# srihari-humbarwadi/retinanet-tensorflow2.x

Hardware: AMD Instinct MI355X
Metric: images/sec train, ResNet50-640 RetinaNet data-parallel step (encode + fwd + loss + bwd + clip + all-reduce + SGD/EMA); inference images/s under `infer` (higher is better)
Workload: dtype bf16; 1 GPU; ResNet50-640x640 bf16 training, 32 images/GPU (BASELINE configs[2] shard: global batch 32), resnet_initial frozen, single GPU; global_batch=32, parallelism=dp1, rccl_ranks=1, comm=torch, syncbn_messages=0

## Files before the change

### include/rnet_hip.h

```cpp
#ifndef RNET_HIP_H_
#define RNET_HIP_H_

#include <stddef.h>
#include <stdint.h>

#ifdef __cplusplus
extern "C" {
#endif
#if defined(__GNUC__)
#pragma GCC visibility push(default)
#endif

typedef enum {
  RN_OK = 0,
  RN_EINVAL = -1,
  RN_ENOMEM = -2,
  RN_EHIP = -3,
  RN_ECOMM = -4,
  RN_EUNSUPPORTED = -5
} rn_status;

enum { RN_DT_F32 = 0, RN_DT_BF16 = 1 };
enum { RN_ACT_NONE = 0, RN_ACT_RELU = 1, RN_ACT_RELU6 = 2, RN_ACT_SWISH = 3 };
enum { RN_FUSION_FAST_ATTENTION = 1, RN_FUSION_FAST_CHANNEL_ATTENTION = 2 };
// ... 100 lines not shown

typedef struct {
  const void* x;
  const void* w;
  void* y;
  const float* scale;
  const float* shift;
  const void* residual;
  int32_t N, H, W, Cin, pix_stride, Ho, Wo, Cout;
  float* bn_partial;
  const float* bias;
  int32_t w_terms;
  int32_t w_pair;
  const void* bn_bwd_y;
  const float* bn_bwd_fwd;
} rn_conv_segment;

typedef struct {
  int32_t R, S, stride_h, stride_w, pad_top, pad_left;
  int32_t act;
  int32_t out_dtype;
  int32_t num_segments;
  rn_conv_segment seg[RN_CONV_MAX_SEGMENTS];
  rn_launch_opts opts;
  void* splitk_ws;
  int64_t splitk_ws_bytes;
} rn_conv_problem;

int rn_conv2d_nhwc_fwd(const rn_conv_problem* problem , void* stream);
size_t rn_conv_splitk_workspace_bytes(const rn_conv_problem* problem );
// ... 271 lines not shown
```

### retinanet-tensorflow2.x_amd/csrc/rn_conv.hip

```cpp
#include "rn_conv_dev.h"

template <int BM, int BN, int BK, bool OUT_F32, int STAGES, bool SPLIT>
__global__ void __launch_bounds__(CONV_THREADS, 2) conv_fwd_kernel(const ConvArgs args) {
  static_assert((STAGES >= 3 && STAGES <= 8) || STAGES == 32, "no K loop for this stage count");
  constexpr int WM = 2, WN = 2;
  constexpr int NWAVES = WM * WN;
  constexpr int NTHREADS = 64 * NWAVES;
  constexpr int SLOTS = BK / 8;
  constexpr int RPI = 64 / SLOTS;
  constexpr int A_INSTR = BM / RPI / NWAVES;
  constexpr int B_INSTR = BN / RPI / NWAVES;
  constexpr int WTM = BM / WM, WTN = BN / WN;
  constexpr int TM = WTM / 32, TN = WTN / 32;
  constexpr int KSUB = BK / 16;
  constexpr int A_BYTES = BM * BK * 2, B_BYTES = BN * BK * 2;
  constexpr int STAGE_BYTES = A_BYTES + B_BYTES;
  static_assert(A_INSTR >= 1 && B_INSTR >= 1, "tile too small for the wave count");

  extern __shared__ __attribute__((aligned(16))) char smem[];

  int tile, part = 0;
  {
    const int total = SPLIT ? args.vtotal : args.total_tiles;
    const int bid = blockIdx.x;
// ... 346 lines not shown
        }
#pragma unroll
        for (int q = 0; q < 4; ++q) {
          float t = f4[q] + sbs[q];
          if (round1) t = rn_rb(t);
          if (affine) t = t * ssc[q] + ssf[q];
          if (round2) t = rn_rb(t);
          f4[q] = t;
        }
        v = make_float4(f4[0], f4[1], f4[2], f4[3]);
      } else {
        v = *(const float4*)(cl + rr * BN + ec);
      }
      const long long o = (long long)m * Cout + n;
      if (sg.residual) {
        const uint2 rv = *(const uint2*)(sg.residual + o);
        v.x += rn_bf16_to_f32((uint16_t)(rv.x & 0xffffu));
        v.y += rn_bf16_to_f32((uint16_t)(rv.x >> 16));
        v.z += rn_bf16_to_f32((uint16_t)(rv.y & 0xffffu));
        v.w += rn_bf16_to_f32((uint16_t)(rv.y >> 16));
      }
      {
        float f4[4] = {v.x, v.y, v.z, v.w};
        if (!OUT_F32 && args.act == RN_ACT_SWISH) {
#pragma unroll
          for (int q = 0; q < 4; ++q) f4[q] = rn_rb(f4[q]);
        }
        rn_apply_act_n<4>(f4, args.act);
        v = make_float4(f4[0], f4[1], f4[2], f4[3]);
      }
      if (OUT_F32) {
// ... 253 lines not shown
```

### retinanet-tensorflow2.x_amd/csrc/rn_conv_big_epi.h

```cpp
#ifndef RN_CONV_BIG_EPI_H_
#define RN_CONV_BIG_EPI_H_
#include <type_traits>

#include "rn_conv_dev.h"

#ifdef HALO_PROF
__device__ unsigned long long g_halo_clk[48];
#define EPI_STAMP(k_) if (blockIdx.x == 0 && threadIdx.x == 0) g_halo_clk[k_] = clock64();
#else
#define EPI_STAMP(k_)
#endif

#ifdef HALO_ABLATE
#define EPI_ABLATE HALO_ABLATE
#else
#define EPI_ABLATE 0
#endif

typedef rn_h16 bf16x2_t __attribute__((ext_vector_type(2)));
typedef float f32x2_t __attribute__((ext_vector_type(2)));

__device__ __forceinline__ uint32_t pack2(float lo, float hi) {
  f32x2_t v = {lo, hi};
  bf16x2_t b = __builtin_convertvector(v, bf16x2_t);
  return __builtin_bit_cast(uint32_t, b);
}
typedef short i16x2_t __attribute__((ext_vector_type(2)));
__device__ __forceinline__ uint32_t pk_max_i16(uint32_t a, uint32_t b) {
  return __builtin_bit_cast(uint32_t, __builtin_elementwise_max(__builtin_bit_cast(i16x2_t, a), __builtin_bit_cast(i16x2_t, b)));
}
__device__ __forceinline__ uint32_t pk_min_i16(uint32_t a, uint32_t b) {
  return __builtin_bit_cast(uint32_t, __builtin_elementwise_min(__builtin_bit_cast(i16x2_t, a), __builtin_bit_cast(i16x2_t, b)));
}
__device__ __forceinline__ float bf_lo(uint32_t u) { return rn_lo16(u); }
__device__ __forceinline__ float bf_hi(uint32_t u) { return rn_hi16(u); }

__device__ __forceinline__ int tile_of(int v, int total) {
  const int xcd = v & 7, slot = v >> 3;
  const int q = total >> 3, r = total & 7;
  return (xcd < r ? xcd * (q + 1) : r * (q + 1) + (xcd - r) * q) + slot;
}

template <bool OUT_F32, bool HAS_RES>
__device__ __forceinline__ bool big_bias_in_acc(const ConvArgs& args, const ConvSegDev& sg) {
  if (HAS_RES) return false;
  return sg.bias != nullptr;
}
template <bool OUT_F32, bool HAS_RES, int WM = 2>
__device__ __forceinline__ void big_acc_init(f32x16_t (&acc)[4][2], const ConvArgs& args, int c_si, int c_n0, int wave,
                                             bool with_bias = true) {
// ... 131 lines not shown
    }
#pragma unroll
    for (int q = 0; q < 8; ++q) asm volatile("" : "+v"(sc[q]), "+v"(sf[q]));
    if (BN_BWD) {
#pragma unroll
      for (int q = 0; q < 8; ++q) asm volatile("" : "+v"(mu[q]), "+v"(is[q]));
    }
    EPI_STAMP(12);
    const bool has_res = HAS_RES && sg.residual != nullptr;
    const uint16_t* const side = BN_BWD ? sg.bn_y : sg.residual;
    const bool has_side = BN_BWD ? true : has_res;
    const bool stats = sg.bn_partial != nullptr;
    float st0[8], st1[8];
#pragma unroll
    for (int q = 0; q < 8; ++q) st0[q] = st1[q] = 0.0f;
    char* const ybase = (char*)sg.y + ((long long)(mw0 + rrow) * Cout + nr) * 2;
    const long long row_bytes = (long long)Cout * 2;
    const int act = args.act;
    const bool clamp_lo = act == RN_ACT_RELU || act == RN_ACT_RELU6, clamp_hi = act == RN_ACT_RELU6;
    const bool affine = !BN_BWD && (sg.scale != nullptr || sg.shift != nullptr);
    const bool plain = BN_BWD || (!affine && !has_res && act != RN_ACT_SWISH);
    const bool round2 = affine && has_res;
    uint4 rv[2][LOADS ? 4 : 1];
#define BIG_RES_PREFETCH(buf_, i_)                                                                    \
_Pragma("unroll") for (int pass = 0; pass < (LOADS ? 4 : 0); ++pass) {                              \
  const int m = mw0 + (i_) * 32 + pass * 8 + rrow;                                                  \
  rv[buf_][pass] = make_uint4(0u, 0u, 0u, 0u);                                                      \
  if (has_side && nok && m < M) rv[buf_][pass] = *(const uint4*)(side + (long long)m * Cout + nr);  \
}
    const uint32_t lo2 = clamp_lo ? 0u : 0x80008000u, hi2 = clamp_hi ? RN_SIX_X2 : 0x7fff7fffu;
    auto blocks = [&](auto plain_c, auto stats_c, auto round2_c, auto swish_c) __attribute__((always_inline)) {
      constexpr bool PLAIN = decltype(plain_c)::value;
      constexpr int STATS = decltype(stats_c)::value, ROUND2 = decltype(round2_c)::value, SWISH = decltype(swish_c)::value;
      BIG_RES_PREFETCH(0, 0);
#pragma unroll
      for (int i = 0; i < 4; ++i) {
        EPI_STAMP(13 + 2 * i);
        if (i + 1 < 4) BIG_RES_PREFETCH((i + 1) & 1, i + 1);
        if (FROM_WS) big_epi_rebuild<2>(&acc[i][0], src, i, 0);
#pragma unroll
        for (int j = 0; j < 2; ++j)
#pragma unroll
          for (int g = 0; g < 4; ++g) {
            const int nl = j * 32 + g * 8 + fh * 4;
            uint2 pk;
            pk.x = pack2(acc[i][j][g * 4 + 0], acc[i][j][g * 4 + 1]);
            pk.y = pack2(acc[i][j][g * 4 + 2], acc[i][j][g * 4 + 3]);
            *(uint2*)(patch + fr * 128 + (((nl >> 3) ^ (fr & 7)) << 4) + ((((nl >> 2) ^ (fr >> 3)) & 1) << 3)) = pk;
          }
        EPI_STAMP(14 + 2 * i);
        uint4 vb[4];
#pragma unroll
        for (int pass = 0; pass < 4; ++pass) {
          const int row = pass * 8 + rrow;
          const uint4 t = *(const uint4*)(patch + row * 128 + ((ru ^ (row & 7)) << 4));
          vb[pass] = (pass & 1) ? make_uint4(t.z, t.w, t.x, t.y) : t;
        }
#pragma unroll
        for (int pass = 0; pass < 4; ++pass) {
          const int row = pass * 8 + rrow;
          const uint4 v = vb[pass];
          const int m = mw0 + i * 32 + row;
          if (m < M && nok) {
            uint4 ov;
            if (PLAIN) {
              ov.x = pk_min_i16(pk_max_i16(v.x, lo2), hi2); ov.y = pk_min_i16(pk_max_i16(v.y, lo2), hi2);
              ov.z = pk_min_i16(pk_max_i16(v.z, lo2), hi2); ov.w = pk_min_i16(pk_max_i16(v.w, lo2), hi2);
            } else {
              const uint4 r4 = HAS_RES ? rv[i & 1][LOADS ? pass : 0] : make_uint4(0u, 0u, 0u, 0u);
              float f[8] = {bf_lo(v.x), bf_hi(v.x), bf_lo(v.y), bf_hi(v.y), bf_lo(v.z), bf_hi(v.z), bf_lo(v.w), bf_hi(v.w)};
              const float rr[8] = {bf_lo(r4.x), bf_hi(r4.x), bf_lo(r4.y), bf_hi(r4.y),
                                   bf_lo(r4.z), bf_hi(r4.z), bf_lo(r4.w), bf_hi(r4.w)};
#pragma unroll
              for (int q = 0; q < 8; ++q) f[q] = f[q] * sc[q] + sf[q];
              if (ROUND2 == 1 || (ROUND2 == 2 && round2)) {
#pragma unroll
                for (int q = 0; q < 8; q += 2) {
                  const uint32_t pq = pack2(f[q], f[q + 1]);
                  f[q] = bf_lo(pq); f[q + 1] = bf_hi(pq);
                }
              }
#pragma unroll
              for (int q = 0; q < 8; ++q) f[q] += rr[q];
              if (SWISH == 1 || (SWISH == 2 && act == RN_ACT_SWISH)) {
#pragma unroll
                for (int q = 0; q < 8; ++q) f[q] = rn_swish(rn_rb(f[q]));
              }
              ov.x = pack2(f[0], f[1]); ov.y = pack2(f[2], f[3]); ov.z = pack2(f[4], f[5]); ov.w = pack2(f[6], f[7]);
              ov.x = pk_min_i16(pk_max_i16(ov.x, lo2), hi2); ov.y = pk_min_i16(pk_max_i16(ov.y, lo2), hi2);
              ov.z = pk_min_i16(pk_max_i16(ov.z, lo2), hi2); ov.w = pk_min_i16(pk_max_i16(ov.w, lo2), hi2);
            }
            if (!(EPI_ABLATE & 16) || ov.x == 0x12345678u) *(uint4*)(ybase + (long long)(i * 32 + pass * 8) * row_bytes) = ov;
            if (STATS == 1 || (STATS == 2 && stats)) {
              const float w[8] = {bf_lo(ov.x), bf_hi(ov.x), bf_lo(ov.y), bf_hi(ov.y),
                                  bf_lo(ov.z), bf_hi(ov.z), bf_lo(ov.w), bf_hi(ov.w)};
              if (BN_BWD) {
                const uint4 y4 = rv[i & 1][LOADS ? pass : 0];
                const float yy[8] = {bf_lo(y4.x), bf_hi(y4.x), bf_lo(y4.y), bf_hi(y4.y),
                                     bf_lo(y4.z), bf_hi(y4.z), bf_lo(y4.w), bf_hi(y4.w)};
#pragma unroll
                for (int q = 0; q < 8; ++q) {
                  const float g = (yy[q] * sc[q] + sf[q]) > 0.0f ? w[q] : 0.0f;
                  st0[q] += g;
                  st1[q] += g * ((yy[q] - mu[BN_BWD ? q : 0]) * is[BN_BWD ? q : 0]);
                }
              } else {
#pragma unroll
                for (int q = 0; q < 8; ++q) { st0[q] += w[q]; st1[q] += w[q] * w[q]; }
              }
            }
          }
        }
      }
    };
    typedef std::integral_constant<int, 0> off_t;
    typedef std::integral_constant<int, 1> on_t;
    typedef std::integral_constant<int, 2> runtime_t;
    if constexpr (BN_BWD) {
      blocks(std::true_type{}, on_t{}, off_t{}, off_t{});
    } else if (plain) {
      if (stats) blocks(std::true_type{}, on_t{}, off_t{}, off_t{});
      else blocks(std::true_type{}, off_t{}, off_t{}, off_t{});
    } else if (!stats && act != RN_ACT_SWISH) {
      if (round2) blocks(std::false_type{}, off_t{}, on_t{}, off_t{});
      else blocks(std::false_type{}, off_t{}, off_t{}, off_t{});
    } else {
      blocks(std::false_type{}, runtime_t{}, runtime_t{}, runtime_t{});
    }
    EPI_STAMP(21);
    if (stats) {
#pragma unroll
      for (int q = 0; q < 8; ++q) {
#pragma unroll
        for (int o = 8; o < 64; o <<= 1) {
          st0[q] += __shfl_xor(st0[q], o, 64);
          st1[q] += __shfl_xor(st1[q], o, 64);
        }
      }
      if (rrow == 0 && nok) {
        float* dst = sg.bn_partial + ((long long)(chunk0 >= 0 ? chunk0 : c_m0 / 128) + wave_m) * 2 * Cout + nr;
        *(float4*)(dst) = make_float4(st0[0], st0[1], st0[2], st0[3]);
        *(float4*)(dst + 4) = make_float4(st0[4], st0[5], st0[6], st0[7]);
// ... 58 lines not shown
```

### retinanet-tensorflow2.x_amd/csrc/rn_conv_dev.h

```cpp
#ifndef RN_CONV_DEV_H_
#define RN_CONV_DEV_H_
#include "rn_common.h"

typedef rn_h16 bf16x8_t __attribute__((ext_vector_type(8)));
typedef float f32x16_t __attribute__((ext_vector_type(16)));

#define CONV_THREADS 256

struct ConvSegDev {
  const uint16_t* x;
  const uint16_t* w;
  void* y;
  const float* scale;
  const float* shift;
  const uint16_t* residual;
  float* bn_partial;
  const float* bias;
  const uint16_t* bn_y;
  const float* bn_fwd;
  int N, H, W, Cin, pix_stride, Ho, Wo, Cout;
  int M, tile_begin, n_tiles, CinP;
  int cwrap, halo_pitch;
  int pair_cout, rows;
};


struct ConvArgs {
  int R, S, sh, sw, pt, pl, act, nseg, total_tiles, pad_;
  int split_f, split_s, vtotal, pad2_;
  float* ws;
  ConvSegDev seg[RN_CONV_MAX_SEGMENTS];
};

#define RN_SPLITK_HEADER_BYTES 16384
// ... 30 lines not shown
```

### retinanet-tensorflow2.x_amd/csrc/rn_conv_dispatch.hip

```cpp
#include <algorithm>
#include <map>
#include <mutex>
#include <tuple>

#include "rn_conv_dev.h"

extern "C" int rn_conv_cout_pad(int Cout) { return Cout <= 64 ? 64 : (int)rn_align_up((size_t)Cout, 128); }
extern "C" int rn_conv_cin_pad(int Cin) { return Cin <= 32 ? 32 : (int)rn_align_up((size_t)Cin, 64); }
extern "C" int rn_conv_pair_rows(int Cout) { return Cout > 0 ? 128 * ((Cout + 63) / 64) : 0; }

struct ConvPlanSeg {
  int cols, cols_pad;
  int terms, cin_pad;
  long long M;
  int n_tiles, tile_begin;
  int bn_row_blocks;
};

struct ConvPlan {
  int kid;
  int BM, BN;
  int BK;
  int bal_rows;
  bool deal;
// ... 212 lines not shown
    RN_CHECK_ARG(s.Cout % 4 == 0, "rn_conv2d_nhwc_fwd: segment %d Cout=%d not a multiple of 4", i, s.Cout);
    RN_CHECK_ARG((pl.seg[i].cols_pad <= 64) == (pl.seg[0].cols_pad <= 64), "rn_conv2d_nhwc_fwd: segments mix Cout tile widths");
    RN_CHECK_ARG(!s.w_pair || (pl.kid != 0 && p->out_dtype == RN_DT_F32 && s.w_terms <= 1 && !s.scale && !s.shift &&
                               !s.residual && !s.bn_partial),
                 "rn_conv2d_nhwc_fwd: segment %d: w_pair needs an f32 launch without scale / shift / residual that the 256- / "
                 "512-row kernels take (rn_conv_kernel_id() != 0)", i);
    RN_CHECK_ARG(((uintptr_t)s.x | (uintptr_t)s.w | (uintptr_t)s.y | (uintptr_t)s.residual) % 16 == 0,
                 "rn_conv2d_nhwc_fwd: segment %d tensors must be 16-byte aligned", i);
    RN_CHECK_ARG(pl.seg[i].M < (1ll << 31) && (long long)s.N * s.H * s.W * s.pix_stride * 2 < (1ll << 31),
                 "rn_conv2d_nhwc_fwd: segment %d input exceeds the 2 GiB buffer-addressing limit", i);
    if (s.bn_bwd_y) {
      RN_CHECK_ARG(s.bn_partial && s.bn_bwd_fwd && p->out_dtype == RN_DT_BF16 && !s.scale && !s.shift && !s.bias &&
                       !s.residual && p->act == RN_ACT_NONE && s.Cout % 8 == 0 && (uintptr_t)s.bn_bwd_y % 16 == 0,
                   "rn_conv2d_nhwc_fwd: segment %d: bn_bwd_y needs bn_partial + bn_bwd_fwd on a plain bf16 launch", i);
    }
    RN_CHECK_ARG((s.bn_bwd_y != nullptr) == (p->seg[0].bn_bwd_y != nullptr),
                 "rn_conv2d_nhwc_fwd: bn_bwd_y must be set on all segments or none");
    RN_CHECK_ARG(pl.seg[i].terms <= 3, "rn_conv2d_nhwc_fwd: segment %d w_terms=%d (1..3)", i, s.w_terms);
  }
  RN_CHECK_ARG(p->splitk_ws == nullptr || ((uintptr_t)p->splitk_ws % 16 == 0 && p->splitk_ws_bytes >= 0),
               "rn_conv2d_nhwc_fwd: splitk_ws must be 16-byte aligned");
  return RN_OK;
}

extern "C" int rn_conv2d_nhwc_fwd(const rn_conv_problem* p, void* stream) {
  RN_CHECK_ARG(p != nullptr, "rn_conv2d_nhwc_fwd: null problem");
  RN_CHECK_ARG(p->num_segments >= 1 && p->num_segments <= RN_CONV_MAX_SEGMENTS,
               "rn_conv2d_nhwc_fwd: num_segments=%d", p->num_segments);
  ConvPlan pl;
  conv_plan(p, false, pl);
// ... 2 lines not shown
  ConvArgs a;
  a.R = p->R; a.S = p->S; a.sh = p->stride_h; a.sw = p->stride_w; a.pt = p->pad_top; a.pl = p->pad_left;
  a.act = p->act; a.nseg = p->num_segments;
  a.total_tiles = (int)pl.total_tiles;
  a.pad_ = pl.kid <= 1 ? (pl.fast_div ? 1 : 0) | (pl.deal ? 2 : 0) : 0;
  a.split_f = a.vtotal = a.total_tiles; a.split_s = 1; a.pad2_ = 0; a.ws = nullptr;
  for (int ii = 0; ii < p->num_segments; ++ii) {
    const rn_conv_segment& s = p->seg[pl.order[ii]];
    const ConvPlanSeg& ps = pl.seg[pl.order[ii]];
    ConvSegDev& d = a.seg[ii];
    d.x = (const uint16_t*)s.x; d.w = (const uint16_t*)s.w; d.y = s.y;
    d.scale = s.scale; d.shift = s.shift; d.residual = (const uint16_t*)s.residual;
    d.bn_partial = s.bn_partial;
    d.bn_y = (const uint16_t*)s.bn_bwd_y;
    d.bn_fwd = s.bn_bwd_fwd;
    d.bias = s.bias;
    d.N = s.N; d.H = s.H; d.W = s.W; d.Cin = s.Cin; d.pix_stride = s.pix_stride;
    d.Ho = s.Ho; d.Wo = s.Wo; d.Cout = ps.cols;
    d.pair_cout = s.w_pair ? s.Cout : 0;
    d.rows = pl.bal_rows;
    d.M = (int)ps.M;
    d.tile_begin = ps.tile_begin;
    d.n_tiles = ps.n_tiles;
    d.cwrap = ps.cin_pad;
    d.CinP = ps.terms * ps.cin_pad;
    d.halo_pitch = s.W + 1;
  }

  hipStream_t st = (hipStream_t)stream;
  const bool f32 = p->out_dtype == RN_DT_F32;
// ... 13 lines not shown
```

### retinanet-tensorflow2.x_amd/csrc/rn_core.hip

```cpp
#include "rn_common.h"
#include <string.h>
#include <new>

static thread_local char g_rn_err[512] = "";

void rn_set_error(const char* fmt, ...) {
  va_list ap;
  va_start(ap, fmt);
  vsnprintf(g_rn_err, sizeof(g_rn_err), fmt, ap);
  va_end(ap);
}

extern "C" const char* rn_last_error(void) { return g_rn_err; }

extern "C" int rn_abi_version(void) { return 13; }

extern "C" int rn_storage_dtype(void) {
#ifdef RN_F16
  return 1;
#else
  return 0;
#endif
}

extern "C" int rn_device_ok(void) {
  int n = 0;
  if (hipGetDeviceCount(&n) != hipSuccess || n <= 0) {
    (void)hipGetLastError();
    return 0;
  }
// ... 122 lines not shown
```

### retinanet-tensorflow2.x_amd/retinanet/_C.py

```python
from __future__ import annotations

import ctypes
import logging
import os
from ctypes import (POINTER, Structure, c_char_p, c_float, c_int, c_int32, c_int64, c_longlong, c_size_t, c_uint32,
                    c_uint64, c_void_p)

_HERE = os.path.dirname(os.path.abspath(__file__))
LIB_PATH = os.environ.get("RNET_HIP_LIB") or os.path.join(_HERE, "librnet_hip.so")
LIB_PATH_F16 = os.environ.get("RNET_HIP_LIB_F16") or os.path.join(_HERE, "librnet_hip_f16.so")

RN_DT_F32, RN_DT_BF16 = 0, 1
RN_OK, RN_EINVAL, RN_ENOMEM, RN_EHIP, RN_ECOMM, RN_EUNSUPPORTED = 0, -1, -2, -3, -4, -5
RN_ACT_NONE, RN_ACT_RELU, RN_ACT_RELU6, RN_ACT_SWISH = 0, 1, 2, 3
RN_FUSION_FAST_ATTENTION, RN_FUSION_FAST_CHANNEL_ATTENTION = 1, 2
FUSION_IDS = {"fast_attention": RN_FUSION_FAST_ATTENTION, "fast_channel_attention": RN_FUSION_FAST_CHANNEL_ATTENTION}
RN_CONV_MAX_SEGMENTS = 10
ABI_VERSION = 13
RN_OPT_ADAM, RN_OPT_RMSPROP, RN_OPT_ADAGRAD, RN_OPT_SGD = 1, 2, 3, 4
RN_OPT_AMSGRAD, RN_OPT_CENTERED, RN_OPT_MOMENTUM, RN_OPT_NESTEROV = 1, 2, 4, 8
PRED_W_TERMS = int(os.environ.get("RNET_PRED_W_TERMS", "2"))
ACT_IDS = {None: RN_ACT_NONE, "none": RN_ACT_NONE, "relu": RN_ACT_RELU, "relu6": RN_ACT_RELU6,
           "swish": RN_ACT_SWISH}


class RnetError(RuntimeError):
    pass


class DgradPack(Structure):
    _fields_ = [("w_ohwi", c_void_p), ("w_packed", c_void_p), ("R", c_int32), ("S", c_int32), ("Cin", c_int32),
                ("Cout", c_int32), ("Cout_pad", c_int32), ("pad_", c_int32)]

# ... 26 lines not shown
class OptimRule(Structure):
    _fields_ = [("rule", c_int32), ("flags", c_int32), ("lr", c_float), ("beta1", c_float), ("beta2", c_float),
                ("rho", c_float), ("momentum", c_float), ("epsilon", c_float), ("ema_decay", c_float)]


class Bottleneck64Problem(Structure):
    _fields_ = [("x", c_void_p), ("y", c_void_p), ("w_packed", c_void_p), ("affine", c_void_p), ("N", c_int32), ("H", c_int32),
                ("W", c_int32), ("Cx", c_int32), ("opts", LaunchOpts)]


class ConvSegment(Structure):
    _fields_ = [("x", c_void_p), ("w", c_void_p), ("y", c_void_p), ("scale", c_void_p), ("shift", c_void_p),
                ("residual", c_void_p), ("N", c_int32), ("H", c_int32), ("W", c_int32), ("Cin", c_int32),
                ("pix_stride", c_int32), ("Ho", c_int32), ("Wo", c_int32), ("Cout", c_int32), ("bn_partial", c_void_p),
                ("bias", c_void_p), ("w_terms", c_int32), ("w_pair", c_int32), ("bn_bwd_y", c_void_p),
                ("bn_bwd_fwd", c_void_p)]


class ConvProblem(Structure):
    _fields_ = [("R", c_int32), ("S", c_int32), ("stride_h", c_int32), ("stride_w", c_int32),
                ("pad_top", c_int32), ("pad_left", c_int32), ("act", c_int32), ("out_dtype", c_int32),
                ("num_segments", c_int32), ("seg", ConvSegment * RN_CONV_MAX_SEGMENTS), ("opts", LaunchOpts),
                ("splitk_ws", c_void_p), ("splitk_ws_bytes", c_int64)]


class WgradSegment(Structure):
    _fields_ = [("x", c_void_p), ("dy", c_void_p), ("N", c_int32), ("H", c_int32), ("W", c_int32),
                ("Cin", c_int32), ("Ho", c_int32), ("Wo", c_int32), ("Cout", c_int32),
                ("dy_pix_stride", c_int32), ("x_pix_stride", c_int32)]


# ... 411 lines not shown
```

### retinanet-tensorflow2.x_amd/retinanet/model/train_engine.py

```python
from __future__ import annotations

import ctypes
import os
from typing import NamedTuple

import numpy as np
import torch

from retinanet import _C
from .bottleneck import Bottleneck64, fused_blocks
from .data_parallel import GradientOverlap, SmallMessages
from .forward import (FoldedConvs, FusionState, conv_launch_name, conv_problem, dw_problem, fold_bn, half_activations, maxpool_step,
                      output_view, padded_outputs, split_by_depth, stem_input, stem_pool_partner, stem_pool_step, stem_problem, tensor_readers,
                      topdown_step)

_DT = {"bf16": torch.bfloat16, "f32": torch.float32}
_SEG_DTYPE = np.dtype([("offset", "<i8"), ("size", "<i8"), ("wd", "<i4"), ("bb", "<i4"), ("nb", "<i4"),
                       ("pad", "<i4"), ("bf", "<i8")])


def _hwio_to_ohwi(w):
    return w.permute(3, 0, 1, 2).contiguous()


# ... 12 lines not shown
    frozen: bool = False


class BackwardStep:
    __slots__ = ("run", "side", "writes", "wgrad")

    def __init__(self, run, side=False, writes=(), wgrad=None):
        self.run, self.side, self.writes, self.wgrad = run, side, writes, wgrad

    def __call__(self, st):
        return self.run(st)


class TrainEngine:
    def __init__(self, model, batch_size, frozen_regexes=(), process_group=None, world_size=None, frozen_names=(),
                 launch_opts=None, wide_pred_terms=None, force_dp=None):
        self.model = model
        self.g = model.graph
        self.params_cfg = model.params
        self.B = int(batch_size)
        self.dev = model.device
        env = os.environ.get
        if force_dp is None:
            force_dp = env("RNET_FORCE_DP", "0") == "1"
        if wide_pred_terms is None:
            wide_pred_terms = env("RNET_TRAIN_PRED_W_TERMS") or \
                getattr(getattr(model.params, "training", None), "prediction_weight_planes", None) or 2
        comm_cus = int(env("RNET_COMM_CUS", "8"))
        self.fuse_bn_stats = env("RNET_FUSE_BN_STATS", "1") != "0"
        self.fuse_bn_bwd = env("RNET_FUSE_BN_BWD", "1") != "0"
        self.fuse_bn_bwd_groups = env("RNET_FUSE_BN_BWD", "1") == "2"
        self.side_stream_on = env("RNET_WGRAD_STREAM", "1") != "0"
        cus = env("RNET_WGRAD_CUS", "160,208")
        self._wgrad_cap = tuple(int(v) for v in cus.split(",")) if cus not in ("0", "") else None
        if not self.side_stream_on:
            self._wgrad_cap = None
        if self._wgrad_cap and len(self._wgrad_cap) == 1:
            self._wgrad_cap = (self._wgrad_cap[0], 2 * self._wgrad_cap[0])
        self._wgrad_group_mode = env("RNET_WGRAD_GROUP", "halo")
        self._ab_workspaces = env("RNET_AB_WORKSPACES") == "1"
        self.f16 = half_activations(model.params)
        self.h16 = torch.float16 if self.f16 else torch.bfloat16
        self._DT = {"bf16": self.h16, "f32": torch.float32}
        self.lib = _C.lib(self.f16)
# ... 499 lines not shown
    def _conv_meta(self, p):
        osz = 4 if p.out_dtype == _C.RN_DT_F32 else 2
        dom = True
        for i in range(p.num_segments):
            s = p.seg[i]
            dom = dom and s.Cout > 64 and s.Cin % 64 == 0 and p.out_dtype == _C.RN_DT_BF16
        if id(p) in self._algo:
            flops, byts = self._algo[id(p)]
        else:
            flops = byts = 0
            for i in range(p.num_segments):
                s = p.seg[i]
                flops += 2 * s.N * s.Ho * s.Wo * p.R * p.S * s.Cin * s.Cout
                byts += 2 * s.N * s.H * s.W * s.pix_stride + osz * s.N * s.Ho * s.Wo * s.Cout + 2 * p.R * p.S * s.Cin * s.Cout
                if s.residual:
                    byts += 2 * s.N * s.Ho * s.Wo * s.Cout
        variant = None
        kid = self.lib.rn_conv_kernel_id(ctypes.byref(p))
        has_res = any(p.seg[i].residual for i in range(p.num_segments))
        bnb = bool(p.seg[0].bn_bwd_y)
        tmpl = (f"<{'true' if p.out_dtype == _C.RN_DT_F32 else 'false'}, {'true' if has_res else 'false'}, "
                f"{'true' if bnb else 'false'}>")
        if kid == 2:
            variant = "conv_halo_kernel" + tmpl[:-1] + ", false, 2> (256x256x32, 3x3 halo patch)"
        elif kid == 3:
            variant = "conv_halo_kernel" + tmpl[:-1] + ", false, 4> (512x128x32, 3x3 halo patch)"
        elif kid == 1:
            variant = "conv_big_kernel" + tmpl + " (256x256x32)"
        elif dom:
            variant = "conv_fwd_kernel<128,128,64,bf16>"
        return flops, byts, variant
# ... 322 lines not shown
        lib, B = self.lib, self.B
        self.bwd_steps = []
        self.dgrad_packs = []
        ops = self.ops
        self.dw_flip_packs = []
        plan, done = [], set()
        for op in ops:
            if op["op"] in ("conv", "dwconv"):
                launch = self._launch_ops(op, done)
                if launch:
                    plan.append((op["op"], launch))
            elif op["op"] in ("maxpool", "topdown", "balance", "stem", "se"):
                plan.append((op["op"], op))
        plan.reverse()
        written = set()

        def mark(name):
            first = name not in written
            written.add(name)
            return first

        for kind, item in plan:
            if kind == "conv":
                self._plan_conv_backward(item, mark)
            elif kind == "dwconv":
                self._plan_dw_backward(item, mark)
            elif kind == "se":
                op = item
                x, dy, dx = self.t[op["inp"]], self.grad[op["out"]], self.grad[op["inp"]]
                mark(op["inp"])
                name, se = op["se"], self.g.ses[op["se"]]
                a = (x.data_ptr(), dy.data_ptr(), dx.data_ptr(), B, x.shape[1] * x.shape[2], se["C"],
                     self.Pbf.data_ptr() + 2 * self.bf_off[name + ":w1"],
                     self.Pbf.data_ptr() + 2 * self.bf_off[name + ":w2"], se["se"], self.se_state[op["out"]].data_ptr(),
                     self._pview(name + "/conv2d/kernel", self.G).data_ptr(),
# ... 67 lines not shown
                op = item
                names = op["tensors"]
                dout = [self.grad["bal:" + n] for n in names]
                ins = [self.t[n] for n in names]
                din = [self.grad[n] for n in names]
                for n in names:
                    mark(n)
                nsc = lib.rn_balance_features_bwd_scratch_bytes(len(names), op["mid"], B, ins[0].shape[1], ins[0].shape[2],
                                                                ins[0].shape[3])
                scratch = torch.empty((max(int(nsc), 256),), dtype=torch.uint8, device=self.dev)
                pd, pi, pn = _C.ptr_array(dout), _C.ptr_array(ins), _C.ptr_array(din)
                self._keep += [pd, pi, pn, scratch]
                a = (pd, pi, pn, self.bal_avg.data_ptr(), scratch.data_ptr(), scratch.numel(), len(names), op["mid"], B,
                     ins[0].shape[1], ins[0].shape[2], ins[0].shape[3])
                self.bwd_steps.append(BackwardStep(lambda st, a=a: _C.check(lib.rn_balance_features_bwd(*a, st), "balance_bwd")))
        self._launch_names = {id(q): n for n, q in self.conv_launches}
        self._loss_dy = {k: {lv: self.dy_of[name] for lv, name in self.g.outputs[k].items() if name in self.dy_of}
                         for k in self.g.outputs}
        if self.dgrad_packs:
            arr = (_C.DgradPack * len(self.dgrad_packs))()
            for i, (mptr, k, cin, cout, cw, buf, mode) in enumerate(self.dgrad_packs):
                arr[i].w_ohwi, arr[i].w_packed = mptr, buf.data_ptr()
                arr[i].R, arr[i].S, arr[i].Cin, arr[i].Cout, arr[i].Cout_pad, arr[i].pad_ = k, k, cin, cout, cw, mode
            self._dgrad_pack_items = arr

    def _plan_fused_topdown_backward(self, op, act, mark):
        lib, B, fus = self.lib, self.B, self.fusion_state[id(op)]
        L = len(op["ins"])
        prev_g = prev_coef = None
        for l in range(L):
# ... 146 lines not shown
    def _plan_conv_backward(self, ops, mark):
        lib, B = self.lib, self.B
        if not self._conv_trainable(ops[0]) and not any(self.requires.get(o["inp"]) for o in ops):
            return
        if not self._conv_trainable(ops[0]):
            raise NotImplementedError("backward through a frozen conv that sits above trainable layers")
        live_bn = bool(self._bn_trainable(ops[0]))
        frozen_bn = self._bn_frozen(ops[0])
        if live_bn or frozen_bn:
            grp = self.bn_groups[ops[0]["out"]]
            pb = grp.problem
            for i, op in enumerate(ops):
                s = pb.seg[i]
                s.dz = self.grad[op["out"]].data_ptr()
                if op.get("residual") and self.requires.get(op["residual"]):
                    dres, first = self._grad_target(op["residual"], mark, balanced=False)
                    s.dres, s.dres_accumulate = dres.data_ptr(), 0 if first else 1
            if frozen_bn:
                self.bwd_steps.append(self._bn_frozen_bwd_step(grp))
            else:
                self.bwd_steps.append(self._bn_bwd_step(grp, self.bn_bwd_ws.get(id(pb), grp.ws)))
            dy_of = {op["out"]: grp.dys[i] for i, op in enumerate(ops)}
        else:
            dy_of = {}
            for op in ops:
                if op["out_dtype"] == "f32":
                    shp = list(self.t[op["out"]].shape)
                    shp[3] = (shp[3] + 63) // 64 * 64
                    dyb = torch.zeros(shp, dtype=self.h16, device=self.dev)
                    dy_of[op["out"]] = dyb
# ... 141 lines not shown
                gbuf, first = self._grad_target(op["inp"], mark)
                s = p.seg[i]
                s.x, s.w, s.y = src.data_ptr(), flips[op["dw"]].data_ptr(), gbuf.data_ptr()
                s.scale, s.shift = None, None
                s.residual = None if first else gbuf.data_ptr()
                s.N, s.H, s.W, s.C, s.Ho, s.Wo = B, H, W, d["C"], H, W
            self._keep.append(p)
            self.dw_launches.append(("dw_dgrad:" + "+".join(o["out"] for o in sub), "dgrad", p, ups))

            def dgrad(st, p=p, ups=ups):
                for u in ups:
                    _C.check(lib.rn_upsample_zero2x(*u, st), "rn_upsample_zero2x")
                _C.check(lib.rn_depthwise_conv2d_nhwc_fwd(ctypes.byref(p), st), "dw dgrad")
            self.bwd_steps.append(BackwardStep(dgrad))

    def _bn_bwd_fusable(self, name):
        if not self.fuse_bn_bwd or name in self.bal_src or len(self.readers.get(name, [])) != 1:
            return None
        hit = self._bn_of_tensor.get(name)
        if hit is None:
            return None
        pb, i, o, nseg = hit
        if nseg != 1 and not self.fuse_bn_bwd_groups:
            return None
        if (o["op"] != "conv" or o.get("act") != "relu" or o.get("residual") or
                o.get("survival") is not None or not self._bn_trainable(o) or pb.seg[i].sample_scale):
            return None
        return pb, i

    def _fuse_bn_bwd(self, p, need):
# ... 55 lines not shown
            c = self.g.convs[op["conv"]]
            cin = c["cin"]
            dy = dy_of[op["out"]]
            cw = dy.shape[3]
            cwp = lib.rn_conv_cin_pad(cw)
            if op["conv"] not in packs:
                shape = (lib.rn_conv_cout_pad(4 * cin), 2, 2, cwp) if subpixel else (lib.rn_conv_cout_pad(cin), k, k, cwp)
                packs[op["conv"]] = torch.empty(shape, dtype=self.h16, device=self.dev)
                off, _ = self.p_off[c.get("kvar", op["conv"] + "/kernel")]
                self.dgrad_packs.append((self.P.data_ptr() + 4 * off, k, cin, c["cout"], cwp, packs[op["conv"]],
                                         1 if subpixel else 0))
            x = self._src(op["inp"])
            H, W = x.shape[1], x.shape[2]
            gbuf, first = self._grad_target(op["inp"], mark)
            firsts.append(first)
            src, dst, cout, res = dy, gbuf, cin, None
            if subpixel:
                cout = 4 * cin
                dst = torch.empty((B, dy.shape[1], dy.shape[2], cout), dtype=self.h16, device=self.dev)
                post.append((dst.data_ptr(), gbuf.data_ptr(), B, dy.shape[1], dy.shape[2], cin, 0 if first else 1))
            elif lowres:
                dst = torch.empty((B, dy.shape[1], dy.shape[2], cin), dtype=self.h16, device=self.dev)
                post.append((dst.data_ptr(), gbuf.data_ptr(), B, dy.shape[1], dy.shape[2], cin, H, W, 0 if first else 1))
            else:
                if stride == 2:
                    src, up_args = self._zero_upsampled(dy, H, W)
                    ups.append(up_args)
                res = None if first else gbuf.data_ptr()
            if dst is not gbuf:
                self._keep.append(dst)
            s = p.seg[i]
            s.x, s.w, s.y = src.data_ptr(), packs[op["conv"]].data_ptr(), dst.data_ptr()
            s.scale, s.shift, s.residual = None, None, res
            s.N, s.H, s.W, s.Cin, s.pix_stride = B, src.shape[1], src.shape[2], cw, cw
            s.Ho, s.Wo, s.Cout = dst.shape[1], dst.shape[2], cout
            Ho, Wo = self.tensors[op["out"]][:2]
            fl += 2 * B * Ho * Wo * k * k * cin * c["cout"]
            by += 2 * B * Ho * Wo * c["cout"] + 2 * B * H * W * cin * (2 if res else 1) + 2 * k * k * cin * c["cout"]
        if post_op is None and stride == 1 and all(firsts):
            by += self._fuse_bn_bwd(p, need)
        self._algo[id(p)] = (fl, by)
        self._keep.append(p)
        self.conv_launches.append(("dgrad:" + (need[0].get("group") or need[0]["out"]), p))

        def dgrad(st, p=p, ups=ups, post=post):
            for u in ups:
                _C.check(lib.rn_upsample_zero2x(*u, st), "rn_upsample_zero2x")
            self._launch_conv(p, st, "dgrad")
            for a in post:
                _C.check(post_op[0](*a, st), post_op[1])
        self.bwd_steps.append(BackwardStep(dgrad))

    def refresh_dgrad_weights(self, st):
# ... 255 lines not shown
```

Before: 1139 images/s.

## Fold gated skip-connection gradient into the stride-1 dgrad conv epilogue

For identity skip connections with a ReLU join, the residual-branch gradient is no longer written separately by the BN backward. Instead the downstream dgrad conv epilogue reads the join gradient, masks it with the ReLU activation bitmask, and adds it as a residual. This removes a separate gradient write and accumulate pass over the skip tensor. The cost is extra gate-bit loads and DPP shuffles in the epilogue, new template variants, and stricter planning constraints enforced with asserts.

```diff
diff --git a/include/rnet_hip.h b/include/rnet_hip.h
--- a/include/rnet_hip.h
+++ b/include/rnet_hip.h
@@ -138,6 +138,7 @@
   int32_t w_pair;
   const void* bn_bwd_y;
   const float* bn_bwd_fwd;
+  const uint8_t* residual_gate;
 } rn_conv_segment;
 
 typedef struct {
diff --git a/retinanet-tensorflow2.x_amd/csrc/rn_conv.hip b/retinanet-tensorflow2.x_amd/csrc/rn_conv.hip
--- a/retinanet-tensorflow2.x_amd/csrc/rn_conv.hip
+++ b/retinanet-tensorflow2.x_amd/csrc/rn_conv.hip
@@ -384,7 +384,12 @@
       }
       const long long o = (long long)m * Cout + n;
       if (sg.residual) {
-        const uint2 rv = *(const uint2*)(sg.residual + o);
+        uint2 rv = *(const uint2*)(sg.residual + o);
+        if (!OUT_F32 && sg.res_gate) {
+          const uint32_t bits = (uint32_t)sg.res_gate[o >> 3] >> (n & 4);
+          rv.x &= ((bits & 1u) ? 0xffffu : 0u) | ((bits & 2u) ? 0xffff0000u : 0u);
+          rv.y &= ((bits & 4u) ? 0xffffu : 0u) | ((bits & 8u) ? 0xffff0000u : 0u);
+        }
         v.x += rn_bf16_to_f32((uint16_t)(rv.x & 0xffffu));
         v.y += rn_bf16_to_f32((uint16_t)(rv.x >> 16));
         v.z += rn_bf16_to_f32((uint16_t)(rv.y & 0xffffu));
diff --git a/retinanet-tensorflow2.x_amd/csrc/rn_conv_big_epi.h b/retinanet-tensorflow2.x_amd/csrc/rn_conv_big_epi.h
--- a/retinanet-tensorflow2.x_amd/csrc/rn_conv_big_epi.h
+++ b/retinanet-tensorflow2.x_amd/csrc/rn_conv_big_epi.h
@@ -34,6 +34,11 @@
 }
 __device__ __forceinline__ float bf_lo(uint32_t u) { return rn_lo16(u); }
 __device__ __forceinline__ float bf_hi(uint32_t u) { return rn_hi16(u); }
+
+template <int L>
+__device__ __forceinline__ uint32_t quad_lane(uint32_t v) {
+  return (uint32_t)__builtin_amdgcn_mov_dpp((int)v, L * 0x55, 0xf, 0xf, true);
+}
 
 __device__ __forceinline__ int tile_of(int v, int total) {
   const int xcd = v & 7, slot = v >> 3;
@@ -195,24 +200,49 @@
     float st0[8], st1[8];
 #pragma unroll
     for (int q = 0; q < 8; ++q) st0[q] = st1[q] = 0.0f;
-    char* const ybase = (char*)sg.y + ((long long)(mw0 + rrow) * Cout + nr) * 2;
+    char* const ybase = BN_BWD ? (char*)sg.y + ((long long)(mw0 + rrow) * Cout + nr) * 2 : nullptr;
     const long long row_bytes = (long long)Cout * 2;
+    char* const y_w = BN_BWD ? nullptr : (char*)sg.y + ((long long)mw0 * Cout + nw0) * 2;
+    const uint16_t* const side_w = !BN_BWD && has_side ? side + ((long long)mw0 * Cout + nw0) : nullptr;
+    const int lane_off = BN_BWD ? 0 : (rrow * Cout + ru * 8) * 2;
     const int act = args.act;
     const bool clamp_lo = act == RN_ACT_RELU || act == RN_ACT_RELU6, clamp_hi = act == RN_ACT_RELU6;
     const bool affine = !BN_BWD && (sg.scale != nullptr || sg.shift != nullptr);
     const bool plain = BN_BWD || (!affine && !has_res && act != RN_ACT_SWISH);
     const bool round2 = affine && has_res;
     uint4 rv[2][LOADS ? 4 : 1];
+    const bool has_gate = HAS_RES && has_res && sg.res_gate != nullptr;
 #define BIG_RES_PREFETCH(buf_, i_)                                                                    \
+if (GATE == 1) {                                                                                    \
+  gw[buf_] = 0xffffffffu;                                                                           \
+  {                                                                                                 \
+    const int go = glane + (i_) * 4 * Cout;                                                         \
+    if (go + 4 <= gend) {                                                                           \
+      __builtin_memcpy(&gw[buf_], gate + (uint32_t)go, 4);    \
+    } else if (go < gend) {                                                                         \
+      uint32_t t = 0u;                                                                              \
+      _Pragma("unroll") for (int k = 0; k < 4; ++k) if (go + k < gend) t |= (uint32_t)gate[(uint32_t)(go + k)] << (8 * k); \
+      gw[buf_] = t;                                                                                 \
+    }                                                                                               \
+  }                                                                                                 \
+}                                                                                                   \
 _Pragma("unroll") for (int pass = 0; pass < (LOADS ? 4 : 0); ++pass) {                              \
   const int m = mw0 + (i_) * 32 + pass * 8 + rrow;                                                  \
   rv[buf_][pass] = make_uint4(0u, 0u, 0u, 0u);                                                      \
-  if (has_side && nok && m < M) rv[buf_][pass] = *(const uint4*)(side + (long long)m * Cout + nr);  \
+  if (has_side && nok && m < M)                                                                     \
+    rv[buf_][pass] = *(const uint4*)(BN_BWD ? (const char*)(side + (long long)m * Cout + nr)          \
+                                            : (const char*)side_w + (uint32_t)(lane_off + ((i_) * 32 + pass * 8) * (Cout * 2))); \
 }
     const uint32_t lo2 = clamp_lo ? 0u : 0x80008000u, hi2 = clamp_hi ? RN_SIX_X2 : 0x7fff7fffu;
-    auto blocks = [&](auto plain_c, auto stats_c, auto round2_c, auto swish_c) __attribute__((always_inline)) {
+    auto blocks = [&](auto plain_c, auto stats_c, auto round2_c, auto swish_c, auto gate_c) __attribute__((always_inline)) {
       constexpr bool PLAIN = decltype(plain_c)::value;
       constexpr int STATS = decltype(stats_c)::value, ROUND2 = decltype(round2_c)::value, SWISH = decltype(swish_c)::value;
+      constexpr int GATE = HAS_RES && !PLAIN ? decltype(gate_c)::value : 0;
+      const long long gate0 = ((long long)mw0 * Cout + nw0) >> 3, gate_left = (((long long)sg.M * Cout) >> 3) - gate0;
+      const uint8_t* const gate = GATE == 1 ? sg.res_gate + gate0 : nullptr;
+      const int gend = (int)(gate_left < 0 ? 0 : gate_left > 0x3fffffff ? 0x3fffffff : gate_left);
+      const int glane = (((rrow + 8 * (ru & 3)) * Cout) >> 3) + 4 * (ru >> 2), gsh = 8 * (ru & 3);
+      uint32_t gw[2];
       BIG_RES_PREFETCH(0, 0);
 #pragma unroll
       for (int i = 0; i < 4; ++i) {
@@ -242,6 +272,10 @@
           const int row = pass * 8 + rrow;
           const uint4 v = vb[pass];
           const int m = mw0 + i * 32 + row;
+          uint32_t bits = 0xffu;
+          if (GATE == 1)
+            bits = (pass == 0 ? quad_lane<0>(gw[i & 1]) : pass == 1 ? quad_lane<1>(gw[i & 1]) :
+                    pass == 2 ? quad_lane<2>(gw[i & 1]) : quad_lane<3>(gw[i & 1])) >> gsh;
           if (m < M && nok) {
             uint4 ov;
             if (PLAIN) {
@@ -250,10 +284,15 @@
             } else {
               const uint4 r4 = HAS_RES ? rv[i & 1][LOADS ? pass : 0] : make_uint4(0u, 0u, 0u, 0u);
               float f[8] = {bf_lo(v.x), bf_hi(v.x), bf_lo(v.y), bf_hi(v.y), bf_lo(v.z), bf_hi(v.z), bf_lo(v.w), bf_hi(v.w)};
-              const float rr[8] = {bf_lo(r4.x), bf_hi(r4.x), bf_lo(r4.y), bf_hi(r4.y),
-                                   bf_lo(r4.z), bf_hi(r4.z), bf_lo(r4.w), bf_hi(r4.w)};
-#pragma unroll
-              for (int q = 0; q < 8; ++q) f[q] = f[q] * sc[q] + sf[q];
+              float rr[8] = {bf_lo(r4.x), bf_hi(r4.x), bf_lo(r4.y), bf_hi(r4.y),
+                             bf_lo(r4.z), bf_hi(r4.z), bf_lo(r4.w), bf_hi(r4.w)};
+              if (GATE == 2 && has_gate) bits = sg.res_gate[((long long)m * Cout + nr) >> 3];
+              if (GATE != 0) {
+#pragma unroll
+                for (int q = 0; q < 8; ++q) rr[q] = ((bits >> q) & 1u) ? rr[q] : 0.0f;
+              }
+#pragma unroll
+              for (int q = 0; q < 8; ++q) f[q] = GATE == 1 ? f[q] + 0.0f : f[q] * sc[q] + sf[q];
               if (ROUND2 == 1 || (ROUND2 == 2 && round2)) {
 #pragma unroll
                 for (int q = 0; q < 8; q += 2) {
@@ -271,7 +310,8 @@
               ov.x = pk_min_i16(pk_max_i16(ov.x, lo2), hi2); ov.y = pk_min_i16(pk_max_i16(ov.y, lo2), hi2);
               ov.z = pk_min_i16(pk_max_i16(ov.z, lo2), hi2); ov.w = pk_min_i16(pk_max_i16(ov.w, lo2), hi2);
             }
-            if (!(EPI_ABLATE & 16) || ov.x == 0x12345678u) *(uint4*)(ybase + (long long)(i * 32 + pass * 8) * row_bytes) = ov;
+            if (!(EPI_ABLATE & 16) || ov.x == 0x12345678u) *(uint4*)(BN_BWD ? ybase + (long long)(i * 32 + pass * 8) * row_bytes
+                                                                           : y_w + (uint32_t)(lane_off + (i * 32 + pass * 8) * (Cout * 2))) = ov;
             if (STATS == 1 || (STATS == 2 && stats)) {
               const float w[8] = {bf_lo(ov.x), bf_hi(ov.x), bf_lo(ov.y), bf_hi(ov.y),
                                   bf_lo(ov.z), bf_hi(ov.z), bf_lo(ov.w), bf_hi(ov.w)};
@@ -298,15 +338,16 @@
     typedef std::integral_constant<int, 1> on_t;
     typedef std::integral_constant<int, 2> runtime_t;
     if constexpr (BN_BWD) {
-      blocks(std::true_type{}, on_t{}, off_t{}, off_t{});
+      blocks(std::true_type{}, on_t{}, off_t{}, off_t{}, off_t{});
     } else if (plain) {
-      if (stats) blocks(std::true_type{}, on_t{}, off_t{}, off_t{});
-      else blocks(std::true_type{}, off_t{}, off_t{}, off_t{});
-    } else if (!stats && act != RN_ACT_SWISH) {
-      if (round2) blocks(std::false_type{}, off_t{}, on_t{}, off_t{});
-      else blocks(std::false_type{}, off_t{}, off_t{}, off_t{});
+      if (stats) blocks(std::true_type{}, on_t{}, off_t{}, off_t{}, off_t{});
+      else blocks(std::true_type{}, off_t{}, off_t{}, off_t{}, off_t{});
+    } else if (!stats && act != RN_ACT_SWISH && !(has_gate && affine)) {
+      if (round2) blocks(std::false_type{}, off_t{}, on_t{}, off_t{}, off_t{});
+      else if (has_gate) blocks(std::false_type{}, off_t{}, off_t{}, off_t{}, on_t{});
+      else blocks(std::false_type{}, off_t{}, off_t{}, off_t{}, off_t{});
     } else {
-      blocks(std::false_type{}, runtime_t{}, runtime_t{}, runtime_t{});
+      blocks(std::false_type{}, runtime_t{}, runtime_t{}, runtime_t{}, runtime_t{});
     }
     EPI_STAMP(21);
     if (stats) {
diff --git a/retinanet-tensorflow2.x_amd/csrc/rn_conv_dev.h b/retinanet-tensorflow2.x_amd/csrc/rn_conv_dev.h
--- a/retinanet-tensorflow2.x_amd/csrc/rn_conv_dev.h
+++ b/retinanet-tensorflow2.x_amd/csrc/rn_conv_dev.h
@@ -18,6 +18,7 @@
   const float* bias;
   const uint16_t* bn_y;
   const float* bn_fwd;
+  const uint8_t* res_gate;
   int N, H, W, Cin, pix_stride, Ho, Wo, Cout;
   int M, tile_begin, n_tiles, CinP;
   int cwrap, halo_pitch;
diff --git a/retinanet-tensorflow2.x_amd/csrc/rn_conv_dispatch.hip b/retinanet-tensorflow2.x_amd/csrc/rn_conv_dispatch.hip
--- a/retinanet-tensorflow2.x_amd/csrc/rn_conv_dispatch.hip
+++ b/retinanet-tensorflow2.x_amd/csrc/rn_conv_dispatch.hip
@@ -250,6 +250,8 @@
                        !s.residual && p->act == RN_ACT_NONE && s.Cout % 8 == 0 && (uintptr_t)s.bn_bwd_y % 16 == 0,
                    "rn_conv2d_nhwc_fwd: segment %d: bn_bwd_y needs bn_partial + bn_bwd_fwd on a plain bf16 launch", i);
     }
+    RN_CHECK_ARG(!s.residual_gate || (s.residual && p->out_dtype == RN_DT_BF16 && s.Cout % 8 == 0),
+                 "rn_conv2d_nhwc_fwd: segment %d: residual_gate needs a bf16 launch with a residual input and Cout %% 8 == 0", i);
     RN_CHECK_ARG((s.bn_bwd_y != nullptr) == (p->seg[0].bn_bwd_y != nullptr),
                  "rn_conv2d_nhwc_fwd: bn_bwd_y must be set on all segments or none");
     RN_CHECK_ARG(pl.seg[i].terms <= 3, "rn_conv2d_nhwc_fwd: segment %d w_terms=%d (1..3)", i, s.w_terms);
@@ -282,6 +284,7 @@
     d.bn_partial = s.bn_partial;
     d.bn_y = (const uint16_t*)s.bn_bwd_y;
     d.bn_fwd = s.bn_bwd_fwd;
+    d.res_gate = (const uint8_t*)s.residual_gate;
     d.bias = s.bias;
     d.N = s.N; d.H = s.H; d.W = s.W; d.Cin = s.Cin; d.pix_stride = s.pix_stride;
     d.Ho = s.Ho; d.Wo = s.Wo; d.Cout = ps.cols;
diff --git a/retinanet-tensorflow2.x_amd/csrc/rn_core.hip b/retinanet-tensorflow2.x_amd/csrc/rn_core.hip
--- a/retinanet-tensorflow2.x_amd/csrc/rn_core.hip
+++ b/retinanet-tensorflow2.x_amd/csrc/rn_core.hip
@@ -13,7 +13,7 @@
 
 extern "C" const char* rn_last_error(void) { return g_rn_err; }
 
-extern "C" int rn_abi_version(void) { return 13; }
+extern "C" int rn_abi_version(void) { return 14; }
 
 extern "C" int rn_storage_dtype(void) {
 #ifdef RN_F16
diff --git a/retinanet-tensorflow2.x_amd/retinanet/_C.py b/retinanet-tensorflow2.x_amd/retinanet/_C.py
--- a/retinanet-tensorflow2.x_amd/retinanet/_C.py
+++ b/retinanet-tensorflow2.x_amd/retinanet/_C.py
@@ -16,7 +16,7 @@
 RN_FUSION_FAST_ATTENTION, RN_FUSION_FAST_CHANNEL_ATTENTION = 1, 2
 FUSION_IDS = {"fast_attention": RN_FUSION_FAST_ATTENTION, "fast_channel_attention": RN_FUSION_FAST_CHANNEL_ATTENTION}
 RN_CONV_MAX_SEGMENTS = 10
-ABI_VERSION = 13
+ABI_VERSION = 14
 RN_OPT_ADAM, RN_OPT_RMSPROP, RN_OPT_ADAGRAD, RN_OPT_SGD = 1, 2, 3, 4
 RN_OPT_AMSGRAD, RN_OPT_CENTERED, RN_OPT_MOMENTUM, RN_OPT_NESTEROV = 1, 2, 4, 8
 PRED_W_TERMS = int(os.environ.get("RNET_PRED_W_TERMS", "2"))
@@ -73,7 +73,7 @@
                 ("residual", c_void_p), ("N", c_int32), ("H", c_int32), ("W", c_int32), ("Cin", c_int32),
                 ("pix_stride", c_int32), ("Ho", c_int32), ("Wo", c_int32), ("Cout", c_int32), ("bn_partial", c_void_p),
                 ("bias", c_void_p), ("w_terms", c_int32), ("w_pair", c_int32), ("bn_bwd_y", c_void_p),
-                ("bn_bwd_fwd", c_void_p)]
+                ("bn_bwd_fwd", c_void_p), ("residual_gate", c_void_p)]
 
 
 class ConvProblem(Structure):
diff --git a/retinanet-tensorflow2.x_amd/retinanet/model/train_engine.py b/retinanet-tensorflow2.x_amd/retinanet/model/train_engine.py
--- a/retinanet-tensorflow2.x_amd/retinanet/model/train_engine.py
+++ b/retinanet-tensorflow2.x_amd/retinanet/model/train_engine.py
@@ -50,7 +50,7 @@
 
 class TrainEngine:
     def __init__(self, model, batch_size, frozen_regexes=(), process_group=None, world_size=None, frozen_names=(),
-                 launch_opts=None, wide_pred_terms=None, force_dp=None):
+                 launch_opts=None, wide_pred_terms=None, force_dp=None, gated_skip=True):
         self.model = model
         self.g = model.graph
         self.params_cfg = model.params
@@ -64,6 +64,7 @@
                 getattr(getattr(model.params, "training", None), "prediction_weight_planes", None) or 2
         comm_cus = int(env("RNET_COMM_CUS", "8"))
         self.fuse_bn_stats = env("RNET_FUSE_BN_STATS", "1") != "0"
+        self.gated_skip = bool(gated_skip)
         self.fuse_bn_bwd = env("RNET_FUSE_BN_BWD", "1") != "0"
         self.fuse_bn_bwd_groups = env("RNET_FUSE_BN_BWD", "1") == "2"
         self.side_stream_on = env("RNET_WGRAD_STREAM", "1") != "0"
@@ -593,7 +594,7 @@
                 flops += 2 * s.N * s.Ho * s.Wo * p.R * p.S * s.Cin * s.Cout
                 byts += 2 * s.N * s.H * s.W * s.pix_stride + osz * s.N * s.Ho * s.Wo * s.Cout + 2 * p.R * p.S * s.Cin * s.Cout
                 if s.residual:
-                    byts += 2 * s.N * s.Ho * s.Wo * s.Cout
+                    byts += 2 * s.N * s.Ho * s.Wo * s.Cout + (s.N * s.Ho * s.Wo * s.Cout // 8 if s.residual_gate else 0)
         variant = None
         kid = self.lib.rn_conv_kernel_id(ctypes.byref(p))
         has_res = any(p.seg[i].residual for i in range(p.num_segments))
@@ -946,11 +947,15 @@
                 plan.append((op["op"], op))
         plan.reverse()
         written = set()
+        self._gated_pending, self.gated_joins = {}, []
 
         def mark(name):
+            held = [x for x, (z, _) in self._gated_pending.items() if z == name]
+            assert not held, f"gradient of {name} is written while the gated skip gradient of {held} still reads it"
             first = name not in written
             written.add(name)
             return first
+        mark.written = written
 
         for kind, item in plan:
             if kind == "conv":
@@ -1048,6 +1053,7 @@
                 a = (pd, pi, pn, self.bal_avg.data_ptr(), scratch.data_ptr(), scratch.numel(), len(names), op["mid"], B,
                      ins[0].shape[1], ins[0].shape[2], ins[0].shape[3])
                 self.bwd_steps.append(BackwardStep(lambda st, a=a: _C.check(lib.rn_balance_features_bwd(*a, st), "balance_bwd")))
+        assert not self._gated_pending, f"gated residual joins without their data-gradient launch: {list(self._gated_pending)}"
         self._launch_names = {id(q): n for n, q in self.conv_launches}
         self._loss_dy = {k: {lv: self.dy_of[name] for lv, name in self.g.outputs[k].items() if name in self.dy_of}
                          for k in self.g.outputs}
@@ -1224,6 +1230,9 @@
                 s = pb.seg[i]
                 s.dz = self.grad[op["out"]].data_ptr()
                 if op.get("residual") and self.requires.get(op["residual"]):
+                    if self._gated_skip_join(pb, i, op, mark):
+                        self._gated_pending[op["residual"]] = (op["out"], s.act_mask)
+                        continue
                     dres, first = self._grad_target(op["residual"], mark, balanced=False)
                     s.dres, s.dres_accumulate = dres.data_ptr(), 0 if first else 1
             if frozen_bn:
@@ -1395,6 +1404,24 @@
                 _C.check(lib.rn_depthwise_conv2d_nhwc_fwd(ctypes.byref(p), st), "dw dgrad")
             self.bwd_steps.append(BackwardStep(dgrad))
 
+    def _gated_skip_join(self, pb, i, op, mark):
+        x = op["residual"]
+        s = pb.seg[i]
+        if not self.gated_skip or op["act"] not in ("relu", "relu6") or s.sample_scale or x in self.bal_src:
+            return False
+        if not all(pb.seg[j].act_mask for j in range(pb.num_segments)) or self.tensors[x][2] % 8 != 0:
+            return False
+        if x in mark.written or x in self._gated_pending:
+            return False
+        readers = self.readers.get(x, [])
+        if len(readers) != 2 or sum(1 for o, role in readers if o is op and role == "residual") != 1:
+            return False
+        (a, role), = [(o, r) for o, r in readers if not (o is op and r == "residual")]
+        if role != "inp" or a["op"] != "conv" or a["out"] in self._bneck_skip or not self._conv_trainable(a):
+            return False
+        order = {id(o): n for n, o in enumerate(self.ops)}
+        return self.g.convs[a["conv"]]["stride"] == 1 and order[id(a)] < order[id(op)]
+
     def _bn_bwd_fusable(self, name):
         if not self.fuse_bn_bwd or name in self.bal_src or len(self.readers.get(name, [])) != 1:
             return None
@@ -1480,6 +1507,9 @@
             H, W = x.shape[1], x.shape[2]
             gbuf, first = self._grad_target(op["inp"], mark)
             firsts.append(first)
+            gated = self._gated_pending.pop(op["inp"], None)
+            assert gated is None or (first and post_op is None and stride == 1), \
+                f"gated skip gradient of {op['inp']}: its data-gradient launch is not a first-writer stride-1 launch"
             src, dst, cout, res = dy, gbuf, cin, None
             if subpixel:
                 cout = 4 * cin
@@ -1498,11 +1528,15 @@
             s = p.seg[i]
             s.x, s.w, s.y = src.data_ptr(), packs[op["conv"]].data_ptr(), dst.data_ptr()
             s.scale, s.shift, s.residual = None, None, res
+            if gated is not None:
+                s.residual, s.residual_gate = self.grad[gated[0]].data_ptr(), gated[1]
+                self.gated_joins.append((gated[0], op["inp"], p, i))
             s.N, s.H, s.W, s.Cin, s.pix_stride = B, src.shape[1], src.shape[2], cw, cw
             s.Ho, s.Wo, s.Cout = dst.shape[1], dst.shape[2], cout
             Ho, Wo = self.tensors[op["out"]][:2]
             fl += 2 * B * Ho * Wo * k * k * cin * c["cout"]
-            by += 2 * B * Ho * Wo * c["cout"] + 2 * B * H * W * cin * (2 if res else 1) + 2 * k * k * cin * c["cout"]
+            by += 2 * B * Ho * Wo * c["cout"] + 2 * B * H * W * cin * (2 if s.residual else 1) + 2 * k * k * cin * c["cout"]
+            by += B * H * W * cin // 8 if s.residual_gate else 0
         if post_op is None and stride == 1 and all(firsts):
             by += self._fuse_bn_bwd(p, need)
         self._algo[id(p)] = (fl, by)
```

Result: no change. 1142 images/s, median of 6 (+0.3%).
